# terryye/cuda_FlashAttention

Measured on AMD Instinct MI355X. Metric: FA2 fwd+bwd TFLOP/s at (B=4,H=16,N=8192,d=128); % MFMA peak, higher is better.
Workload: dtype bf16; 1 GPU; FA2 forward+backward bf16, (B=4,H=16,N=8192,d=128) per GPU, non-causal (BASELINE configs[2]); flops = 14 B H N^2 d; B=4, H=16, N=8192, d=128, parallelism=head-sharded replicas x1

## Files before the change

cuda_flashattention_amd/csrc/fa2_bwd_bf16.hip:

```cpp
#include <type_traits>

#include "fa2_regfile.h"
#include "fa2_launch.h"

namespace fa2 {

constexpr float kNoKeyRC = -1.0e30f;
constexpr float kNoKeyLq = 1.0e30f;

template <int D>
__global__ void __launch_bounds__(256) fa2_bwd_delta_kernel(const __bf16* __restrict__ dO,
                                                            const __bf16* __restrict__ O,
                                                            const float* __restrict__ L,
                                                            float* __restrict__ Dv, float* __restrict__ RC,
                                                            size_t rows, int nq, int q_hs, int q_row0, size_t rc_plane,
                                                            float inv_scale)
{
    const size_t r = ((size_t)blockIdx.x * 256 + threadIdx.x) >> 4;
    const int sub = threadIdx.x & 15;
    const size_t head = r / (size_t)nq, i = r % (size_t)nq;
    const size_t row = head * (size_t)q_hs + i;
    const size_t prow = row + (size_t)q_row0;
    float acc = 0.0f;
    if (r < rows) {
#pragma unroll
        for (int c = sub * 8; c < D; c += 128) {
            const bf16x8 a = *reinterpret_cast<const bf16x8*>(dO + row * D + c);
            const bf16x8 b = *reinterpret_cast<const bf16x8*>(O + row * D + c);
#pragma unroll
            for (int e = 0; e < 8; ++e) acc += (float)a[e] * (float)b[e];
        }
    }
#pragma unroll
    for (int off = 8; off >= 1; off >>= 1) acc += __shfl_xor(acc, off, 16);
    if (r < rows && sub == 0) {
        Dv[prow] = acc;
        const float l = L[row];
        RC[prow] = l == -INFINITY ? kNoKeyRC : -l * inv_scale;
        RC[rc_plane + prow] = -acc;
    }
}

constexpr int kBwdRows = 256;
constexpr int kDqWaves = 4;
constexpr int kDqKV = 64;
constexpr int kDkQ = 32;

typedef __attribute__((address_space(3))) void* lptr_t;

#include "fa2_bwd_dq_body.inc"

#define FA2_DQ_CLOBBERS "memory", "vcc", FA2_RF512
#define FA2_DQ_OPS_128 [r0] "v"(roff[0]), [r1] "v"(roff[1]), [r2] "v"(roff[2]), [r3] "v"(roff[3]), [r4] "v"(roff[4]), [r5] "v"(roff[5]), \
    [r6] "v"(roff[6]), [r7] "v"(roff[7]), [t0] "v"(toff[0]), [t1] "v"(toff[1]), [t2] "v"(toff[2]), [t3] "v"(toff[3]), [t4] "v"(toff[4]),     \
    [t5] "v"(toff[5]), [t6] "v"(toff[6]), [t7] "v"(toff[7])
#define FA2_DQ_OPS_64 [r0] "v"(roff[0]), [r1] "v"(roff[1]), [r2] "v"(roff[2]), [r3] "v"(roff[3]), [t0] "v"(toff[0]), [t1] "v"(toff[1]),    \
    [t2] "v"(toff[2]), [t3] "v"(toff[3])

constexpr int kBwdRegFile = RF512;

template <int D, int BUF, bool MASKED>
__device__ __forceinline__ void dq_body(const uint32_t (&roff)[D / 16], const uint32_t (&toff)[D / 16], float c2, float lq0, float lq1,
                                        const f32x16& nd0, const f32x16& nd1, int hi0, int hi1, int hp0, int hp1)
{
#define FA2_DQ_CASE(DD, B, M)                                                                                                      \
    if constexpr (D == DD && BUF == B && MASKED == bool(M))                                                                          \
        asm volatile(FA2_DQ_BODY_D##DD##_B##B##_M##M : : FA2_DQ_OPS_##DD, [c2] "s"(c2), [lq0] "v"(lq0), [lq1] "v"(lq1), [nd0] "v"(nd0), \
                     [nd1] "v"(nd1), [hi0] "v"(hi0), [hi1] "v"(hi1), [hp0] "v"(hp0), [hp1] "v"(hp1) : FA2_DQ_CLOBBERS);
    FA2_DQ_CASE(128, 0, 0) FA2_DQ_CASE(128, 1, 0) FA2_DQ_CASE(128, 2, 0) FA2_DQ_CASE(128, 0, 1) FA2_DQ_CASE(128, 1, 1) FA2_DQ_CASE(128, 2, 1)
    FA2_DQ_CASE(64, 0, 0) FA2_DQ_CASE(64, 1, 0) FA2_DQ_CASE(64, 2, 0) FA2_DQ_CASE(64, 0, 1) FA2_DQ_CASE(64, 1, 1) FA2_DQ_CASE(64, 2, 1)
// ... 361 lines not shown
        } else {
            dkdv_body<D, buf, 0, false>(roff, toff, rcadr, c2, 0, 0, 0);
            dkdv_body<D, buf, 1, false>(roff, toff, rcadr, c2, 0, 0, 0);
        }
    };

    for (int t = t0; t < tend; t += 2) {
        tile(std::integral_constant<int, 0>{}, t);
        tile(std::integral_constant<int, 1>{}, t + 1);
    }
    }

    asm volatile("s_waitcnt lgkmcnt(0)" ::: "memory");
    mfma_acc_settle();
    static_for<2>([&](auto KB) {
        constexpr int kb = decltype(KB)::value;
        const int key = kw0 + 32 * kb + ki;
        char* dKk = (char*)p.dK + slab + (size_t)(key < N ? key : 0) * ROWB;
        char* dVk = (char*)p.dV + slab + (size_t)(key < N ? key : 0) * ROWB;
        static_for<4 * DT>([&](auto G) {
            constexpr int dt = decltype(G)::value / 4, g = decltype(G)::value % 4;
            constexpr int RK = A_DK + 16 * (kb * DT + dt) + 4 * g, RV = A_DV + 16 * (kb * DT + dt) + 4 * g;
            bf16x4 a, b;
            a[0] = (__bf16)(aread<RK>() * p.scale); a[1] = (__bf16)(aread<RK + 1>() * p.scale);
            a[2] = (__bf16)(aread<RK + 2>() * p.scale); a[3] = (__bf16)(aread<RK + 3>() * p.scale);
            b[0] = (__bf16)aread<RV>(); b[1] = (__bf16)aread<RV + 1>();
            b[2] = (__bf16)aread<RV + 2>(); b[3] = (__bf16)aread<RV + 3>();
            if (key < N) {
                *reinterpret_cast<bf16x4*>(dKk + 2 * (32 * dt + 8 * g + 4 * h)) = a;
                *reinterpret_cast<bf16x4*>(dVk + 2 * (32 * dt + 8 * g + 4 * h)) = b;
            }
        });
    });
}

template <int D, bool CAUSAL>
__global__ void __launch_bounds__(256, 1) __attribute__((amdgpu_num_vgpr(60))) fa2_bwd_dkdv_kernel(BwdArgs p)
{
    const int ncb = (p.Nk + kDkKeys - 1) / kDkKeys;
    int kvhead, cb;
    map_block(blockIdx.x, p.BH / p.kv_group, ncb, kvhead, cb);
    bwd_dkdv_impl<D, CAUSAL>(p, kvhead, cb);
}

template <int D, bool CAUSAL>
__global__ void __launch_bounds__(256, 1) __attribute__((amdgpu_num_vgpr(60))) fa2_bwd_dkdv_varlen_kernel(VarlenBwdArgs v)
{
    int kvhead, idx;
    map_block(blockIdx.x, v.a.BH / v.a.kv_group, v.n_key_items, kvhead, idx);
    const VarlenItem it = uniform_item(v.key_items, idx);
    bwd_dkdv_impl<D, CAUSAL>(bwd_varlen_view<D>(v.a, it), kvhead, it.block);
}

template <int D, bool CAUSAL>
static hipError_t launch_bwd_one(const BwdArgs& a, hipStream_t stream)
{
    const size_t rows = (size_t)a.BH * a.Nq;
    hipError_t e = hipSuccess;
    if (a.phases & 1) {
        hipLaunchKernelGGL((fa2_bwd_delta_kernel<D>), dim3((unsigned)((rows * 16 + 255) / 256)), dim3(256), 0,
                           stream, (const __bf16*)a.dO, (const __bf16*)a.O, a.L, a.D, a.RC, rows, a.Nq, a.q_hs, a.q_row0,
                           (size_t)a.BH * a.q_hs, 1.0f / a.scale);
        e = hipGetLastError();
        if (e != hipSuccess) return e;
    }
    const int nb = (a.Nq + kBwdRows - 1) / kBwdRows;
    constexpr int lds_dq = 3 * 2 * kDqKV * D * 2;
    constexpr int lds_dk = kDkKeys * D * 2 + 2 * (2 * 2 * kDkQ * D * 2 + 512);
    if (a.phases & 2) {
        e = launch_lds<fa2_bwd_dq_kernel<D, CAUSAL>>(dim3((unsigned)(nb * a.BH)), dim3(256), lds_dq, stream, a);
        if (e != hipSuccess) return e;
    }
    if (a.phases & 4) {
        const int ncb = (a.Nk + kDkKeys - 1) / kDkKeys;
        e = launch_lds<fa2_bwd_dkdv_kernel<D, CAUSAL>>(dim3((unsigned)(ncb * (a.BH / a.kv_group))), dim3(256), lds_dk, stream, a);
    }
    return e;
}

template <int D, bool CAUSAL>
static hipError_t launch_bwd_varlen_one(const VarlenBwdArgs& v, hipStream_t stream)
{
    const BwdArgs& a = v.a;
    const size_t rows = (size_t)a.BH * a.q_hs;
    hipLaunchKernelGGL((fa2_bwd_delta_kernel<D>), dim3((unsigned)((rows * 16 + 255) / 256)), dim3(256), 0, stream,
                       (const __bf16*)a.dO, (const __bf16*)a.O, a.L, a.D, a.RC, rows, a.q_hs, a.q_hs, 0, rows, 1.0f / a.scale);
    hipError_t e = hipGetLastError();
    if (e != hipSuccess) return e;
    constexpr int lds_dq = 3 * 2 * kDqKV * D * 2;
    constexpr int lds_dk = kDkKeys * D * 2 + 2 * (2 * 2 * kDkQ * D * 2 + 512);
    e = launch_lds<fa2_bwd_dq_varlen_kernel<D, CAUSAL>>(dim3((unsigned)(v.n_row_items * a.BH)), dim3(256), lds_dq, stream, v);
    if (e != hipSuccess) return e;
    return launch_lds<fa2_bwd_dkdv_varlen_kernel<D, CAUSAL>>(dim3((unsigned)(v.n_key_items * (a.BH / a.kv_group))), dim3(256), lds_dk,
                                                            stream, v);
}

hipError_t launch_bwd_varlen_bf16(const VarlenBwdArgs& v, hipStream_t stream)
{
    const BwdArgs& a = v.a;
    if (a.kv_group < 1 || a.BH % a.kv_group != 0 || v.n_row_items < 1 || v.n_key_items < 1 || !v.row_items || !v.key_items)
        return hipErrorInvalidValue;
    if (a.d == 128) return a.causal ? launch_bwd_varlen_one<128, true>(v, stream) : launch_bwd_varlen_one<128, false>(v, stream);
    if (a.d == 64) return a.causal ? launch_bwd_varlen_one<64, true>(v, stream) : launch_bwd_varlen_one<64, false>(v, stream);
    return hipErrorInvalidValue;
}

hipError_t launch_bwd_bf16(const BwdArgs& a, hipStream_t stream)
{
    if (a.kv_group < 1 || a.BH % a.kv_group != 0) return hipErrorInvalidValue;
    if (a.d == 128) return a.causal ? launch_bwd_one<128, true>(a, stream) : launch_bwd_one<128, false>(a, stream);
    if (a.d == 64) return a.causal ? launch_bwd_one<64, true>(a, stream) : launch_bwd_one<64, false>(a, stream);
    return hipErrorInvalidValue;
}

}
```

cuda_flashattention_amd/csrc/fa2_bwd_fused.hip:

```cpp
#include <cstdlib>
#include <cstring>
#include <type_traits>

#include "fa2_regfile.h"
#include "fa2_launch.h"

namespace fa2 {

#include "fa2_bwd_fused_body.inc"

typedef __attribute__((address_space(3))) void* fused_lptr_t;

#ifndef FA2_FUSED_DSKEY
#define FA2_FUSED_DSKEY(row) (((row) >> 1) & 7)
#endif

#ifndef FA2_FUSED_DIAG
#define FA2_FUSED_DIAG 0
#endif

constexpr int kFusedRegFile = RF512;

#define FA2_FUSED_CLOBBERS "memory", "vcc", FA2_RF512
#define FA2_FUSED_OPS_128 [r0] "v"(roff[0]), [r1] "v"(roff[1]), [r2] "v"(roff[2]), [r3] "v"(roff[3]), [r4] "v"(roff[4]), [r5] "v"(roff[5]),  \
    [r6] "v"(roff[6]), [r7] "v"(roff[7]), [t0] "v"(toff[0]), [t1] "v"(toff[1]), [t2] "v"(toff[2]), [t3] "v"(toff[3]), [t4] "v"(toff[4]),   \
    [t5] "v"(toff[5]), [t6] "v"(toff[6]), [t7] "v"(toff[7]), [rc] "v"(rcv), [c2] "s"(c2)
#define FA2_FUSED_OPS_64 [r0] "v"(roff[0]), [r1] "v"(roff[1]), [r2] "v"(roff[2]), [r3] "v"(roff[3]), [t0] "v"(toff[0]), [t1] "v"(toff[1]),    \
    [t2] "v"(toff[2]), [t3] "v"(toff[3]), [rc] "v"(rcv), [c2] "s"(c2)

struct FusedStep {
    __amdgpu_buffer_rsrc_t drs, lrs, qrs, grs, rcrs, ctl;
    uint32_t dso, lso, qso, rcso, pvo, mso;
    int need, pval;
};
#define FA2_FUSED_STEP(TEXT, DD, ...)                                                                                                 \
    asm volatile(TEXT                                                                                                                 \
                 : [err] "+s"(err)                                                                                                    \
                 : FA2_FUSED_OPS_##DD, [vm] "i"(VMW), [dqv] "v"(dqv), [drs] "s"(f.drs), [dso] "s"(f.dso), [lrs] "s"(f.lrs), [lso] "s"(f.lso), \
                   [mw] "s"(mw), [mw2] "s"(mw2), [qrs] "s"(f.qrs), [grs] "s"(f.grs), [rcrs] "s"(f.rcrs), [qso] "s"(f.qso),               \
                   [rcso] "s"(f.rcso), [dvo] "v"(dvo), [rcvo] "v"(rcvo), [wv] "s"(wv), [ctl] "s"(f.ctl), [pvo] "s"(f.pvo),               \
                   [mso] "s"(f.mso), [need] "s"(f.need), [pval] "s"(f.pval) __VA_ARGS__                                                \
                 : FA2_FUSED_CLOBBERS, "s12", "s13", "scc", "exec", "m0", "v39")
template <int D, int BUF, int PAR, int VMW, bool MASKED>
__device__ __forceinline__ void fused_cbody(const uint32_t (&roff)[D / 16], const uint32_t (&toff)[D / 16], uint32_t rcv, float c2, uint32_t dqv,
                                            uint32_t dvo, uint32_t rcvo, uint32_t mw, uint32_t mw2, int wv, const FusedStep& f, int& err,
                                            int lo0 = 0, int lo1 = 0)
{
#define FA2_FUSED_CASE(TAG, DD, B, P)                                                                                                 \
    if constexpr (D == DD && BUF == B && PAR == P && MASKED) FA2_FUSED_STEP(FA2_FUSED##TAG##_MBODY_B##B##_P##P, DD, , [lo0] "v"(lo0), [lo1] "v"(lo1)); \
    if constexpr (D == DD && BUF == B && PAR == P && !MASKED) FA2_FUSED_STEP(FA2_FUSED##TAG##_CBODY_B##B##_P##P, DD);
#define FA2_FUSED_CASES(TAG, DD) \
    FA2_FUSED_CASE(TAG, DD, 0, 0) FA2_FUSED_CASE(TAG, DD, 0, 1) FA2_FUSED_CASE(TAG, DD, 1, 0) FA2_FUSED_CASE(TAG, DD, 1, 1) FA2_FUSED_CASE(TAG, DD, 2, 0) FA2_FUSED_CASE(TAG, DD, 2, 1)
    FA2_FUSED_CASES(, 128) FA2_FUSED_CASES(64, 64)
#undef FA2_FUSED_CASES
#undef FA2_FUSED_CASE
}

template <int BUF, int PAR, int VMW>
__device__ __forceinline__ void fused_body(const uint32_t (&roff)[8], const uint32_t (&toff)[8], uint32_t rcv, float c2)
{
#define FA2_FUSED_CASE(B, P) \
    if constexpr (BUF == B && PAR == P) asm volatile(FA2_FUSED_BODY_B##B##_P##P : : FA2_FUSED_OPS_128, [vm] "i"(VMW) : FA2_FUSED_CLOBBERS);
    FA2_FUSED_CASE(0, 0) FA2_FUSED_CASE(0, 1) FA2_FUSED_CASE(1, 0) FA2_FUSED_CASE(1, 1) FA2_FUSED_CASE(2, 0) FA2_FUSED_CASE(2, 1)
#undef FA2_FUSED_CASE
}

template <int DQT>
__device__ __forceinline__ void fused_dq_atomic(__amdgpu_buffer_rsrc_t rs, uint32_t voff, uint32_t soff)
{
    asm volatile(
        "s_add_u32 s12, %2, 4096\n\ts_add_u32 s13, %2, 8192\n\ts_add_u32 s14, %2, 12288\n\t"
// ... 52 lines not shown
constexpr int g_hook_fault = 0, g_hook_grid = 0;
#define FA2_HOOK_NOTE_GRID(n) ((void)0)
#endif

__device__ __forceinline__ int fused_ctl_ints(int BH, int ncb) { return kCtlHeadmap + 16 * (BH + kHmPad) + 9 * BH * ncb; }

__device__ __forceinline__ int fused_load_sc1(const int* p)
{
    int v;
    asm volatile("global_load_dword %0, %1, off sc1\n\ts_waitcnt vmcnt(0)" : "=v"(v) : "v"(p) : "memory");
    return v;
}
__device__ __forceinline__ void fused_seen_set(int v)
{
    asm volatile("v_mov_b32 v39, %0" : : "s"(v) : "v39");
}

__device__ __forceinline__ int fused_lane_id() { return (int)__builtin_amdgcn_mbcnt_hi(~0u, __builtin_amdgcn_mbcnt_lo(~0u, 0u)); }
template <int OFF>
__device__ __forceinline__ int fused_mail_read(uint32_t lds_addr)
{
    int v;
    asm volatile("v_mov_b32 %0, %1\n\tds_read_b32 %0, %0 offset:%c2\n\ts_waitcnt lgkmcnt(0)" : "=&v"(v) : "s"(lds_addr), "i"(OFF) : "memory");
    return __builtin_amdgcn_readfirstlane(v);
}

__device__ __forceinline__ void fused_store_flag(int* p, int v)
{
    asm volatile("global_store_dword %0, %1, off" : : "v"(p), "v"(v) : "memory");
}

__device__ __forceinline__ bool fused_spin_over(int* ctl, int spins)
{
    if (spins > kSpinLimit) {
        atomicExch(ctl + kCtlError, 1);
        return true;
    }
    return (spins & 1023) == 0 && fused_load_sc1(ctl + kCtlError) != 0;
}

template <bool CHAIN, bool CAUSAL, bool RAGGED = false, bool RECT = false, int HD = 128>
__global__ void __launch_bounds__(256, 1) __attribute__((amdgpu_num_vgpr(39))) fa2_bwd_fused_kernel(FusedArgs fp)
{
    static_assert(CHAIN || !RAGGED, "the atomics form has no ragged variant");
    static_assert(!RECT || (CHAIN && !CAUSAL && !RAGGED), "rectangular blocks: chained, unmasked, aligned");
    static_assert(HD == 128 || (HD == 64 && CHAIN && !RECT), "head_dim 64: chained, square");
    extern __shared__ __attribute__((aligned(16))) char smem[];
    const BwdArgs& p = fp.b;
    constexpr int D = HD, ROWB = 2 * D, KS = D / 16, DT = D / 32;
    constexpr int DQW = 128;
    constexpr int TROWS = 32;
    constexpr bool W = D == 128;
    constexpr int QRING = W ? FA2_FUSED_QRING : FA2_FUSED64_QRING, BUFB = W ? FA2_FUSED_BUFB : FA2_FUSED64_BUFB,
                  DSB = W ? FA2_FUSED_DSB : FA2_FUSED64_DSB, LDSB = W ? FA2_FUSED_LDS : FA2_FUSED64_LDS;
    constexpr int CPR = D / 8, RPI = 64 / CPR, NINS = TROWS / RPI;
    constexpr int VF = W ? FA2_FUSED_VF : FA2_FUSED64_VF, DQT = W ? FA2_FUSED_DQT : FA2_FUSED64_DQT,
                  ROFFK = W ? FA2_FUSED_ROFFK : FA2_FUSED64_ROFFK, DSWR = W ? FA2_FUSED_DSWR : FA2_FUSED64_DSWR,
                  DSRD = W ? FA2_FUSED_DSRD : FA2_FUSED64_DSRD, KT = W ? FA2_FUSED_KT : FA2_FUSED64_KT;
    constexpr int VMW = CHAIN ? (W ? 4 : 2) : 63;
    int* const mail = reinterpret_cast<int*>(smem + LDSB);
    const uint32_t mail_addr = __builtin_amdgcn_readfirstlane((uint32_t)(uintptr_t)smem) + LDSB;

    const int tid = threadIdx.x;
    const int lane = tid & 63;
    const int wave = __builtin_amdgcn_readfirstlane(tid >> 6);
    const int ki = lane & 31;
    const int h = lane >> 5;
    const int N = p.Nk;
    const int NP = RAGGED ? fp.npad : N;
    const int NQ = RECT ? p.Nq : N;
    const int NPQ = RECT ? NQ : NP;
    const int QHS = RECT ? p.q_hs : N, KHS = RECT ? p.k_hs : N;
    const int QR0 = RECT ? p.q_row0 : 0;
    const int ncb = NP / 256;
    const int ntiles = NPQ / TROWS;
    const int niter = ((ntiles + 1 + 5) / 6) * 6;
    const float c2 = p.scale * kLog2e;
    const size_t rc_plane = (size_t)p.BH * (RECT ? QHS : NP);

    const uint32_t lbase = (uint32_t)(uintptr_t)smem;
    const int trq = (lane & 15) >> 2, trp = lane & 3, trcb = (lane >> 4) & 1;
    uint32_t roff[KS], toff[2 * DT];
#pragma unroll
    for (int s = 0; s < KS; ++s) roff[s] = lbase + QRING + lds_off<D>(ki, 2 * s + h);
#pragma unroll
    for (int dt = 0; dt < DT; ++dt)
#pragma unroll
        for (int jj = 0; jj < 2; ++jj)
            toff[2 * dt + jj] = lbase + QRING + lds_off<D>(8 * jj + 4 * h + trq, 4 * dt + 2 * trcb + (trp >> 1)) + 8 * (trp & 1);
    const uint32_t rcv = lbase + QRING + 2 * TROWS * ROWB + 16 * h;
    static_for<KS>([&](auto S) {
        constexpr int sidx = decltype(S)::value;
        vset<kFusedRegFile, CL_TOP, ROFFK + sidx>(lbase + lds_off<D>(ki + 64 * wave, 2 * sidx + h));
    });
    const int ecol = W ? wave : (wave & 1), ekey0 = W ? 0 : 128 * (wave >> 1);
    static_for<2>([&](auto JJ) {
        constexpr int jj = decltype(JJ)::value;
        vset<kFusedRegFile, CL_TOP, KT + jj>(lbase + ekey0 * ROWB + lds_off<D>(8 * jj + 4 * h + trq, 4 * ecol + 2 * trcb + (trp >> 1)) + 8 * (trp & 1));
        const int row = 8 * jj + 4 * h + trq;
        vset<kFusedRegFile, CL_TOP, DSRD + jj>(lbase + DSB + (ekey0 + row) * 64 + 8 * ((4 * trcb + trp) ^ FA2_FUSED_DSKEY(row)));
    });
    static_for<4>([&](auto C) {
        constexpr int c = decltype(C)::value;
        vset<kFusedRegFile, CL_TOP, DSWR + c>(lbase + DSB + (64 * wave + ki) * 64 + 8 * (((2 * c) | h) ^ FA2_FUSED_DSKEY(ki)));
    });
    const int doff = lds_dma_off<D>(wave * RPI, lane);
    const uint32_t dqv = CHAIN ? (uint32_t)(wave * 4096 + lane * 16) : (uint32_t)(((4 * h) * D + 32 * wave + ki) * 4);
// ... 64 lines not shown

    auto next_unit_loads = [&]() {
        if constexpr (CHAIN) {
            take_ticket();
            __syncthreads();
            const int hn = fused_mail_read<0>(mail_addr);
            if (hn >= 0) issue_unit_loads(hn, fused_mail_read<4>(mail_addr));
        }
    };
    next_unit_loads();

    for (;;) {
#ifdef FA2_FUSED_STATS
        const uint64_t s_pull = __builtin_readcyclecounter();
#endif
        int head, cb, err0 = 0;
        if constexpr (CHAIN) {
            head = fused_mail_read<0>(mail_addr);
            cb = fused_mail_read<4>(mail_addr);
            err0 = fused_mail_read<8>(mail_addr);
            if (head < 0) break;
        } else {
            map_block(blockIdx.x, p.BH, ncb, head, cb);
            issue_unit_loads(head, cb);
        }
        const size_t slab = (size_t)head * QHS * ROWB;
        const char* Qh = (const char*)p.Q + slab;
        const char* Gh = (const char*)p.dO + slab;
        const int kw0 = cb * 256 + wave * 64;
        {
            const u32x4 z = {0u, 0u, 0u, 0u};
            static_for<4 * DT>([&](auto T) { azero16<kFusedRegFile, CL_ACC, 16 * decltype(T)::value>(z); });
        }

        const auto q_rsrc = __builtin_amdgcn_make_buffer_rsrc((void*)Qh, 0, NQ * ROWB, 0x00020000);
        const auto g_rsrc = __builtin_amdgcn_make_buffer_rsrc((void*)Gh, 0, NQ * ROWB, 0x00020000);
        const int rcoff = (int)(((wave == 0 ? 0 : rc_plane) + (size_t)head * (RECT ? QHS : NP) + QR0 + (fused_lane_id() & 31)) * 4);
        auto stage = [&](int t, int buf) {
            char* b = smem + QRING + buf * BUFB;
#pragma unroll
            for (int j = wave; j < 2 * NINS; j += 4) {
                const int which = j / NINS, piece = j % NINS;
                const int soff = (t * TROWS + piece * RPI) * ROWB;
                __builtin_amdgcn_raw_ptr_buffer_load_lds(which ? g_rsrc : q_rsrc, (fused_lptr_t)(b + which * (TROWS * ROWB) + piece * 1024),
                                                         16, doff, soff, 0, 0);
            }
            if (wave < 2 && fused_lane_id() < 32)
                __builtin_amdgcn_raw_ptr_buffer_load_lds(rc_rsrc, (fused_lptr_t)(b + 2 * TROWS * ROWB + wave * 128), 4, rcoff, t * TROWS * 4, 0, 0);
        };
        const int n_u = CAUSAL ? ntiles - 8 * cb : ntiles;
        const int niter_u = CAUSAL ? ((n_u + 1 + 5) / 6) * 6 : niter;
        const bool ragged_unit = RAGGED && !CAUSAL && cb == ncb - 1;
        const int first_masked = CAUSAL ? ((n_u - 8) / 6) * 6 : (ragged_unit ? 0 : niter_u);
        auto tl = [&](int u) { return CAUSAL ? ntiles - 1 - u : u; };
        stage(tl(0), 0);
#ifdef FA2_FUSED_PREFILL
        stage(tl(1), 1);
        stage(tl(2), 2);
#endif
        fused_dq_zero<DQT>();
        asm volatile("s_waitcnt vmcnt(0)" ::: "memory");
        __syncthreads();
        if constexpr (W) asm volatile(FA2_FUSED_PRO : : FA2_FUSED_OPS_128, [vm] "i"(VMW) : FA2_FUSED_CLOBBERS);
        else asm volatile(FA2_FUSED64_PRO : : FA2_FUSED_OPS_64, [vm] "i"(VMW) : FA2_FUSED_CLOBBERS);

        const auto dq_rsrc = __builtin_amdgcn_make_buffer_rsrc((void*)(fp.dQacc + (size_t)head * NPQ * DQW), 0, NPQ * DQW * 4, 0x00020000);
        int* const mine = prog_base + head * ncb + cb;
        const int* const prev = mine - 1;
        const int prev_off = (int)((prev - fp.ctl) * 4);
        const int mine_off = (int)((mine - fp.ctl) * 4);
        if constexpr (CHAIN) fused_seen_set(0);
        int err = err0;
#ifdef FA2_FUSED_STATS
        int st_steps = 0, st_polls = 0, st_cycles = 0;
        const uint64_t u0 = __builtin_readcyclecounter();
#endif

        const auto null_rsrc = __builtin_amdgcn_make_buffer_rsrc((void*)fp.dQacc, 0, 0, 0x00020000);
        const bool hp_unit = cb > 0;
        const auto lrs_unit = hp_unit && !(FA2_FUSED_DIAG & 2) ? dq_rsrc : null_rsrc;
        auto step = [&](auto BUF, auto PAR, auto MASKED, auto FAST_, int t) {
            constexpr int buf = decltype(BUF)::value, par = decltype(PAR)::value;
            constexpr bool masked = decltype(MASKED)::value;
            constexpr bool FAST = decltype(FAST_)::value;
            if constexpr (CHAIN && FAST) {
                FusedStep f;
                f.drs = dq_rsrc;
                f.lrs = lrs_unit;
                f.dso = (uint32_t)(tl(t - 1) * TROWS * DQW * 4);
                f.lso = (uint32_t)(tl(t) * TROWS * DQW * 4);
                f.qrs = q_rsrc; f.grs = g_rsrc; f.rcrs = rc_rsrc; f.ctl = ctl_rsrc;
                f.qso = (uint32_t)(tl(t + 1) * TROWS * ROWB + wave * 1024);
                f.rcso = (uint32_t)(tl(t + 1) * TROWS * 4);
                f.pvo = (uint32_t)prev_off; f.mso = (uint32_t)mine_off;
                f.need = (hp_unit && !err && !(FA2_FUSED_DIAG & 1)) ? t + 1 : (int)0x80000000;
                f.pval = t;
#ifdef FA2_TEST_HOOKS
                if (fp.fault && cb == 1) f.pval = 0;
#endif
                fused_cbody<D, buf, par, VMW, false>(roff, toff, rcv, c2, dqv, (uint32_t)doff, (uint32_t)rcoff, lbase + QRING + wave * 1024,
                                                  lbase + QRING + wave * 128, wave, f, err, 0, 0);
            } else if constexpr (CHAIN) {
                FusedStep f;
                const bool live = t >= 1 && t <= n_u;
                const bool more = t + 1 < n_u;
                const bool has_prev = t < n_u && cb > 0;
                f.drs = live ? dq_rsrc : null_rsrc;
                f.lrs = has_prev && !(FA2_FUSED_DIAG & 2) ? dq_rsrc : null_rsrc;
                f.dso = (uint32_t)__builtin_amdgcn_readfirstlane(tl(t - 1) * TROWS * DQW * 4);
                f.lso = (uint32_t)__builtin_amdgcn_readfirstlane(tl(t) * TROWS * DQW * 4);
                f.qrs = q_rsrc; f.grs = g_rsrc; f.rcrs = rc_rsrc; f.ctl = ctl_rsrc;
                f.qso = more ? (uint32_t)(tl(t + 1) * TROWS * ROWB + wave * 1024) : 0x40000000u;
                f.rcso = more ? (uint32_t)(tl(t + 1) * TROWS * 4) : 0x40000000u;
                f.pvo = (uint32_t)prev_off; f.mso = (uint32_t)mine_off;
                f.need = (has_prev && !err && !(FA2_FUSED_DIAG & 1)) ? t + 1 : (int)0x80000000;
                f.pval = t < n_u ? t : n_u;
#ifdef FA2_TEST_HOOKS
                if (fp.fault && cb == 1) f.pval = 0;
#endif
                int lo0 = 0, lo1 = 0;
                if constexpr (masked) {
                    const int lane_m = (int)__builtin_amdgcn_mbcnt_hi(~0u, __builtin_amdgcn_mbcnt_lo(~0u, 0u));
                    if constexpr (CAUSAL) {
                        lo0 = kw0 + (lane_m & 31) - 4 * (lane_m >> 5) - TROWS * tl(t);
                        lo1 = lo0 + 32;
                    } else {
                        lo0 = kw0 + (lane_m & 31) < N ? -0x40000000 : 0x40000000;
                        lo1 = kw0 + 32 + (lane_m & 31) < N ? -0x40000000 : 0x40000000;
                    }
                }
#ifdef FA2_FUSED_STATS2
                const uint64_t b0 = __builtin_readcyclecounter();
#endif
                fused_cbody<D, buf, par, VMW, masked>(roff, toff, rcv, c2, dqv, (uint32_t)doff, (uint32_t)rcoff, lbase + QRING + wave * 1024,
                                                   lbase + QRING + wave * 128, wave, f, err, lo0, lo1);
#ifdef FA2_FUSED_STATS2
                st_cycles += (int)(__builtin_readcyclecounter() - b0);
#endif
            } else {
                static_assert(W || CHAIN, "head_dim 64: chained form only");
                stage(t + 1, (buf + 1) % 3);
                if constexpr (W) fused_body<buf, par, VMW>(roff, toff, rcv, c2);
#ifndef FA2_FUSED_NO_DQ
                if (t >= 1 && t <= ntiles) fused_dq_atomic<DQT>(dq_rsrc, dqv, (uint32_t)__builtin_amdgcn_readfirstlane((t - 1) * TROWS * D * 4));
#endif
                fused_dq_zero<DQT>();
            }
        };
        auto six = [&](auto MASKED, auto FAST_, int t) {
            step(std::integral_constant<int, 0>{}, std::integral_constant<int, 0>{}, MASKED, FAST_, t);
            step(std::integral_constant<int, 1>{}, std::integral_constant<int, 1>{}, MASKED, FAST_, t + 1);
            step(std::integral_constant<int, 2>{}, std::integral_constant<int, 0>{}, MASKED, FAST_, t + 2);
            step(std::integral_constant<int, 0>{}, std::integral_constant<int, 1>{}, MASKED, FAST_, t + 3);
            step(std::integral_constant<int, 1>{}, std::integral_constant<int, 0>{}, MASKED, FAST_, t + 4);
            step(std::integral_constant<int, 2>{}, std::integral_constant<int, 1>{}, MASKED, FAST_, t + 5);
        };
        const int fast_end = CHAIN ? n_u - 2 : -1;
        {
            const int plain_end = first_masked;
            int t = 0;
            asm volatile("" : "+s"(t));
            if (t < plain_end) { six(std::false_type{}, std::false_type{}, t); t += 6; }
#pragma unroll 1
            for (; t + 5 <= fast_end && t < plain_end; t += 6) six(std::false_type{}, std::true_type{}, t);
#pragma unroll 1
            for (; t < plain_end; t += 6) six(std::false_type{}, std::false_type{}, t);
            if constexpr (CHAIN && (CAUSAL || RAGGED)) {
#pragma unroll 1
                for (; t < niter_u; t += 6) six(std::true_type{}, std::false_type{}, t);
            }
        }
        asm volatile("s_waitcnt vmcnt(0) lgkmcnt(0)" ::: "memory");
        if constexpr (CHAIN)
            if (err && !err0 && wave == 0 && fused_lane_id() == 0) atomicExch(fp.ctl + kCtlError, 1);
#ifdef FA2_FUSED_STATS
        const uint64_t s_loop = __builtin_readcyclecounter();
#endif
        next_unit_loads();

        mfma_acc_settle();
        const int lane_ep = (int)__builtin_amdgcn_mbcnt_hi(~0u, __builtin_amdgcn_mbcnt_lo(~0u, 0u));
        const int ki_ep = lane_ep & 31, h_ep = lane_ep >> 5;
        static_for<2>([&](auto KB) {
            constexpr int kb = decltype(KB)::value;
            const int key = kw0 + 32 * kb + ki_ep;
            const size_t slab_k = RECT ? (size_t)head * KHS * ROWB : slab;
            char* const dKb = (char*)p.dK + slab_k;
            char* const dVb = (char*)p.dV + slab_k;
            const uint32_t koff = (uint32_t)key * ROWB + 16u * h_ep;
            char* dKk = dKb + koff;
            char* dVk = dVb + koff;
            static_for<2 * DT>([&](auto G) {
                constexpr int dt = decltype(G)::value / 2, gp = decltype(G)::value % 2;
                constexpr int RK = 16 * (kb * DT + dt) + 8 * gp, RV = 32 * DT + RK;
                auto pack4 = [&](float a, float b, float c, float d, float sc) {
                    bf16x4 v;
                    v[0] = (__bf16)(a * sc); v[1] = (__bf16)(b * sc); v[2] = (__bf16)(c * sc); v[3] = (__bf16)(d * sc);
                    return __builtin_bit_cast(u32x2, v);
                };
                auto emit = [&](u32x2 x, u32x2 y, char* dst) {
                    const auto s0 = __builtin_amdgcn_permlane32_swap(x[0], y[0], false, false);
                    const auto s1 = __builtin_amdgcn_permlane32_swap(x[1], y[1], false, false);
                    const u32x4 o = {s0[0], s1[0], s0[1], s1[1]};
#ifdef FA2_FUSED_ST_NT
                    if (!RAGGED || key < N) __builtin_nontemporal_store(o, reinterpret_cast<u32x4*>(dst + 2 * (32 * dt + 16 * gp)));
#else
                    if (!RAGGED || key < N) *reinterpret_cast<u32x4*>(dst + 2 * (32 * dt + 16 * gp)) = o;
#endif
                };
                emit(pack4(aread<RK>(), aread<RK + 1>(), aread<RK + 2>(), aread<RK + 3>(), p.scale),
                     pack4(aread<RK + 4>(), aread<RK + 5>(), aread<RK + 6>(), aread<RK + 7>(), p.scale), dKk);
                emit(pack4(aread<RV>(), aread<RV + 1>(), aread<RV + 2>(), aread<RV + 3>(), 1.0f),
                     pack4(aread<RV + 4>(), aread<RV + 5>(), aread<RV + 6>(), aread<RV + 7>(), 1.0f), dVk);
            });
        });
#ifdef FA2_FUSED_STATS
        if (CHAIN && wave == 0 && fused_lane_id() == 0) {
            atomicAdd(fp.ctl + kCtlError + 1, st_steps);
            atomicAdd(fp.ctl + kCtlError + 2, st_polls);
            atomicAdd((unsigned long long*)(fp.ctl + kCtlError + 4), (unsigned long long)st_cycles);
            atomicAdd((unsigned long long*)(fp.ctl + kCtlError + 6), (unsigned long long)(__builtin_readcyclecounter() - u0));
            int* rec = prog_base + p.BH * ncb + 8 * (head * ncb + cb);
            rec[0] = xcc; rec[1] = st_cycles; rec[2] = (int)(u0 - s_pull); rec[3] = (int)(__builtin_readcyclecounter() - s_loop);
            *(unsigned long long*)(rec + 4) = u0; *(unsigned long long*)(rec + 6) = __builtin_readcyclecounter();
        }
#endif
        if constexpr (!CHAIN) break;
    }
}

__global__ void __launch_bounds__(256) fa2_bwd_fused_dq_out_kernel(const float* __restrict__ acc, __bf16* __restrict__ dQ, size_t n8, float scale,
                                                                    const int* __restrict__ err)
{
    const float poison = (err && *err) ? __builtin_nanf("") : 0.0f;
    const size_t stride = (size_t)gridDim.x * 256;
    for (size_t i = (size_t)blockIdx.x * 256 + threadIdx.x; i < n8; i += stride) {
        const f32x4 a = reinterpret_cast<const f32x4*>(acc)[2 * i], b = reinterpret_cast<const f32x4*>(acc)[2 * i + 1];
        bf16x8 o;
#pragma unroll
        for (int e = 0; e < 4; ++e) { o[e] = (__bf16)(a[e] * scale + poison); o[4 + e] = (__bf16)(b[e] * scale + poison); }
        reinterpret_cast<bf16x8*>(dQ)[i] = o;
    }
}

__global__ void __launch_bounds__(256) fa2_bwd_fused_dq_out_chain_kernel(const float* __restrict__ acc, __bf16* __restrict__ dQ, size_t n4, float scale,
                                                                          const int* __restrict__ err, int N, int NP, int qhs)
{
    const float poison = *err ? __builtin_nanf("") : 0.0f;
    const size_t stride = (size_t)gridDim.x * 256;
    const size_t tiles = (size_t)(NP / 32);
    for (size_t i = (size_t)blockIdx.x * 256 + threadIdx.x; i < n4; i += stride) {
        const f32x4 a = reinterpret_cast<const f32x4*>(acc)[i];
        const int lane = (int)(i & 63), g = (int)((i >> 6) & 3), wave = (int)((i >> 8) & 3);
        const size_t tg = i >> 10, head = tg / tiles;
        const int row = (int)(tg % tiles) * 32 + 8 * g + 4 * (lane >> 5);
        __bf16* o = dQ + (head * (size_t)qhs + row) * 128 + 32 * wave + (lane & 31);
#pragma unroll
        for (int e = 0; e < 4; ++e)
            if (row + e < N) o[(size_t)e * 128] = (__bf16)(a[e] * scale + poison);
    }
}

__global__ void __launch_bounds__(256) fa2_bwd_fused_dq_out_chain64_kernel(const float* __restrict__ acc, __bf16* __restrict__ dQ, size_t n4h, float scale,
                                                                            const int* __restrict__ err, int N, int NP)
{
    const float poison = *err ? __builtin_nanf("") : 0.0f;
    const size_t stride = (size_t)gridDim.x * 256;
    const size_t tiles = (size_t)(NP / 32);
// ... 46 lines not shown
    int dev = 0;
    if (hipGetDevice(&dev) != hipSuccess || dev < 0 || dev >= 64) { if (why) *why = "no current device"; return false; }
    if (!verdict[dev]) {
        hipDeviceProp_t pr;
        if (hipGetDeviceProperties(&pr, dev) != hipSuccess) { if (why) *why = "device properties unavailable"; return false; }
        verdict[dev] = strncmp(pr.gcnArchName, "gfx950", 6) != 0 ? 2 : pr.multiProcessorCount != 256 ? 3 : 1;
    }
    static const char* const text[] = {"", "single five-product kernel (gfx950, 256 CUs: the layout the ordered hand-off was validated on)",
                                       "two kernels: device is not gfx950", "two kernels: device does not expose 256 CUs (partitioned GPU): "
                                       "the ordered hand-off was validated in SPX mode only"};
    if (why) *why = text[verdict[dev]];
    return verdict[dev] == 1;
}

hipError_t bwd_fused_read_error(const int* ctl, int* err, hipStream_t stream)
{
    hipError_t e = hipMemcpyAsync(err, ctl + kCtlError, sizeof(int), hipMemcpyDeviceToHost, stream);
    if (e != hipSuccess) return e;
    return hipStreamSynchronize(stream);
}

hipError_t bwd_fused_clear_error(int* ctl, hipStream_t stream)
{
    return launch_fill_f32(reinterpret_cast<float*>(ctl + kCtlError), 1, 0.0f, stream);
}

size_t bwd_fused_kvpart_bytes(int BH, int N, int d) { return (size_t)2 * BH * N * d * 2; }
size_t bwd_fused_ctl_bytes(int BH, int N) { return (size_t)(kCtlHeadmap + 16 * (BH + kHmPad) + 9 * BH * ((N + 255) / 256)) * sizeof(int); }

template <int HD>
static hipError_t launch_chained_square(bool causal, bool ragged, dim3 grid, int lds, hipStream_t stream, const FusedArgs& fa)
{
    if (causal)
        return ragged ? launch_lds<fa2_bwd_fused_kernel<true, true, true, false, HD>>(grid, dim3(256), lds, stream, fa)
                      : launch_lds<fa2_bwd_fused_kernel<true, true, false, false, HD>>(grid, dim3(256), lds, stream, fa);
    return ragged ? launch_lds<fa2_bwd_fused_kernel<true, false, true, false, HD>>(grid, dim3(256), lds, stream, fa)
                  : launch_lds<fa2_bwd_fused_kernel<true, false, false, false, HD>>(grid, dim3(256), lds, stream, fa);
}

hipError_t launch_bwd_fused_bf16(const BwdArgs& a, float* dQacc, int* ctl, int mode, hipStream_t stream, float* rcpad, void* kvpart)
{
    const int npad = (a.Nk + 255) / 256 * 256;
    const bool ragged = npad != a.Nk;
    const bool rect = a.Nq != a.Nk || a.q_hs != a.Nq || a.k_hs != a.Nk || a.q_row0 != 0;
    if ((a.d != 128 && a.d != 64) || a.Nk < 1 || a.Nq < 1) return hipErrorInvalidValue;
    if (a.d == 64 && (mode != 1 || rect)) return hipErrorInvalidValue;
    if (rect && (mode != 1 || a.causal || ragged || a.Nq % 32 != 0 || a.q_row0 < 0 || a.q_hs < a.q_row0 + a.Nq || a.k_hs < a.Nk))
        return hipErrorInvalidValue;
    if (ragged && (mode != 1 || !rcpad)) return hipErrorInvalidValue;
    const bool grouped = a.kv_group > 1;
    if (a.kv_group < 1 || a.BH % a.kv_group != 0 || (grouped && (mode != 1 || rect || !kvpart))) return hipErrorInvalidValue;
    if (a.causal && (mode != 1 || a.causal_shift != 0)) return hipErrorInvalidValue;
    hipError_t e = hipSuccess;
    if (a.phases & 1) {
        BwdArgs d = a;
        d.phases = 1;
        e = launch_bwd_bf16(d, stream);
        if (e != hipSuccess) return e;
    }
    if (!(a.phases & 8)) return hipSuccess;
    const size_t elems = (size_t)a.BH * (rect ? a.Nq : npad) * 128;
    const int units = a.BH * (npad / 256);
    if (ragged) {
        const size_t n = (size_t)2 * a.BH * npad;
        hipLaunchKernelGGL(fa2_bwd_fused_rcpad_kernel, dim3((unsigned)((n + 255) / 256)), dim3(256), 0, stream, (const float*)a.RC, rcpad,
                           a.BH, a.Nk, npad);
        e = hipGetLastError();
        if (e != hipSuccess) return e;
    }
    FusedArgs fa{a, dQacc, ctl, npad, ragged ? (const float*)rcpad : (const float*)a.RC, g_hook_fault};
    const size_t part_elems = (size_t)a.BH * a.Nk * a.d;
    if (grouped) {
        fa.b.dK = kvpart;
        fa.b.dV = (__bf16*)kvpart + part_elems;
    }
    const int lds = (a.d == 64 ? FA2_FUSED64_LDS : FA2_FUSED_LDS) + 16;
    if (mode == 0) {
        e = launch_fill_f32(dQacc, elems, 0.0f, stream);
        if (e != hipSuccess) return e;
        e = bwd_fused_clear_error(ctl, stream);
        if (e != hipSuccess) return e;
        e = launch_lds<fa2_bwd_fused_kernel<false, false>>(dim3((unsigned)units), dim3(256), lds, stream, fa);
    } else {
        static int cus[64] = {};
        int dev = 0;
        e = hipGetDevice(&dev);
        if (e != hipSuccess) return e;
        if (dev < 0 || dev >= 64) return hipErrorInvalidDevice;
        if (!cus[dev]) {
            e = hipDeviceGetAttribute(&cus[dev], hipDeviceAttributeMultiprocessorCount, dev);
            if (e != hipSuccess) return e;
        }
        e = launch_fill_f32(reinterpret_cast<float*>(ctl), bwd_fused_ctl_bytes(a.BH, a.Nk) / sizeof(float), 0.0f, stream);
        if (e != hipSuccess) return e;
        int avail = cus[dev] - (a.reserve_cus > 0 ? a.reserve_cus : 0);
        if (avail < 1) avail = 1;
        int wgs = units < avail ? units : avail;
        if (g_hook_grid >= 1 && g_hook_grid < wgs) wgs = g_hook_grid;
        FA2_HOOK_NOTE_GRID(wgs);
        const dim3 grid((unsigned)wgs);
        if (rect)
            e = launch_lds<fa2_bwd_fused_kernel<true, false, false, true>>(grid, dim3(256), lds, stream, fa);
        else
            e = a.d == 64 ? launch_chained_square<64>(a.causal, ragged, grid, lds, stream, fa)
                          : launch_chained_square<128>(a.causal, ragged, grid, lds, stream, fa);
    }
    if (e != hipSuccess) return e;
    if (mode == 0)
        hipLaunchKernelGGL(fa2_bwd_fused_dq_out_kernel, dim3(2048), dim3(256), 0, stream, dQacc, (__bf16*)a.dQ, elems / 8, a.scale,
                           (const int*)nullptr);
    else if (a.d == 64)
        hipLaunchKernelGGL(fa2_bwd_fused_dq_out_chain64_kernel, dim3(4096), dim3(256), 0, stream, dQacc, (__bf16*)a.dQ, elems / 8, a.scale,
                           ctl + kCtlError, a.Nk, npad);
    else
        hipLaunchKernelGGL(fa2_bwd_fused_dq_out_chain_kernel, dim3(4096), dim3(256), 0, stream, dQacc, (__bf16*)a.dQ, elems / 4, a.scale,
                           ctl + kCtlError, rect ? a.Nq : a.Nk, rect ? a.Nq : npad, rect ? a.q_hs : a.Nk);
    e = hipGetLastError();
    if (e != hipSuccess || !grouped) return e;
    hipLaunchKernelGGL(fa2_bwd_fused_dkdv_out_kernel, dim3(4096), dim3(256), 0, stream, (const bf16x8*)fa.b.dK, (const bf16x8*)fa.b.dV,
                       (bf16x8*)a.dK, (bf16x8*)a.dV, (size_t)a.Nk * a.d / 8, (size_t)(a.BH / a.kv_group), a.kv_group);
    return hipGetLastError();
}

}
```

cuda_flashattention_amd/csrc/fa2_launch.h:

```cpp
#pragma once
#include <hip/hip_runtime.h>
#include <stddef.h>

namespace fa2 {

struct FwdArgs {
    const void* Q;
    const void* K;
    const void* V;
    void* O;
    float* L;
    float* Oacc;
    float* M;
    int BH, Nq, Nk, d;
    float scale;
    int causal;
    int causal_shift;
    int resume;
    int finalize;
    int q_hs, k_hs;
    int kv_group;
};

hipError_t launch_fwd1_bf16(const FwdArgs& a, hipStream_t stream);

struct VarlenItem {
    int q_row0, k_row0;
    int len_q, len_k;
    int block;
};
struct VarlenFwdArgs { FwdArgs a; const VarlenItem* items; int n_items; };
hipError_t launch_fwd1_varlen_bf16(const VarlenFwdArgs& v, hipStream_t stream);
hipError_t launch_accumulate_bf16(float* acc, const void* src, size_t rows, size_t cols, size_t pitch, int init, hipStream_t stream);
hipError_t launch_finalize_state(const float* Oacc, const float* M, float* L, void* O, size_t rows, int d, hipStream_t stream);

struct FwdFp8Args {
    const void* Q; const void* K; const void* V;
    void* Vt;
    float* kn;
    void* O;
    float* L;
    int BH, N, Npad, d;
    float scale;
    int causal;
    float o_scale;
};
hipError_t launch_fwd_fp8(const FwdFp8Args& a, hipStream_t stream);

struct BwdArgs {
    const void* Q; const void* K; const void* V; const void* O; const void* dO;
    const float* L;
    void* dQ; void* dK; void* dV;
    float* D;
    float* RC;
    int BH, Nq, Nk, d;
    int q_hs, k_hs;
    int q_row0;
    float scale;
    int causal;
    int causal_shift;
    int phases;
    int reserve_cus;
    int kv_group;
};

hipError_t launch_bwd_bf16(const BwdArgs& a, hipStream_t stream);
struct VarlenBwdArgs {
    BwdArgs a;
    const VarlenItem* row_items; const VarlenItem* key_items;
    int n_row_items, n_key_items;
};
hipError_t launch_bwd_varlen_bf16(const VarlenBwdArgs& v, hipStream_t stream);
size_t bwd_fused_ctl_bytes(int BH, int N);
size_t bwd_fused_kvpart_bytes(int BH, int N, int d);
hipError_t launch_bwd_fused_bf16(const BwdArgs& a, float* dQacc, int* ctl, int mode, hipStream_t stream, float* rcpad = nullptr,
                                 void* kvpart = nullptr);
bool bwd_fused_device_ok(const char** why);
hipError_t bwd_fused_read_error(const int* ctl, int* err, hipStream_t stream);
hipError_t bwd_fused_clear_error(int* ctl, hipStream_t stream);

struct F32Args {
    const float* Q; const float* K; const float* V; float* O; float* L;
    const float* dO; float* dQ; float* dK; float* dV; float* D;
    int BH, N, d;
    float scale;
    int causal;
    int phases;
    int Nk;
    float* M;
    int resume, finalize;
};
hipError_t launch_fwd_f32(const F32Args& a, hipStream_t stream);
hipError_t launch_bwd_f32(const F32Args& a, hipStream_t stream);

template <auto K, typename A>
inline hipError_t launch_lds(dim3 grid, dim3 block, int lds, hipStream_t stream, const A& arg)
{
    static bool done[64] = {};
    int dev = 0;
    hipError_t e = hipGetDevice(&dev);
    if (e != hipSuccess) return e;
    if (dev < 0 || dev >= 64) return hipErrorInvalidDevice;
    if (!done[dev]) {
        e = hipFuncSetAttribute(reinterpret_cast<const void*>(K), hipFuncAttributeMaxDynamicSharedMemorySize, lds);
        if (e != hipSuccess) return e;
        done[dev] = true;
    }
    hipLaunchKernelGGL(K, grid, block, lds, stream, arg);
    return hipGetLastError();
}

hipError_t launch_fa1_f32(const float* Q, const float* K, const float* V, float* O, float* l, float* m, int N, int d, int Bc,
                          hipStream_t stream);

hipError_t launch_fill_f32(float* p, size_t n, float value, hipStream_t stream);
hipError_t launch_mfma_probe(const void* in, float* out, int iters, int blocks, hipStream_t stream);
hipError_t launch_f32_to_bf16(const float* src, void* dst, size_t n, hipStream_t stream);
hipError_t launch_bf16_to_f32(const void* src, float* dst, size_t n, hipStream_t stream);
hipError_t launch_read_clocks(unsigned long long* out, hipStream_t stream);
// ... 3 lines not shown
```

Before: 1311 TFLOP/s.

## Stage fused bwd dK/dV epilogue through LDS and trim tail steps

Rewrites the fused backward kernel's dK/dV epilogue so each wave first packs its accumulators to bf16 with a vector convert, writes them to a swizzled LDS staging area, then reads them back so that global stores become row-contiguous 16-byte writes. The tail six-step group of the chain loop now skips steps beyond the live tile count instead of running padding steps. An optional path (off by default) lets the delta kernel zero the control buffer with extra blocks, removing the separate fill launch. The LDS staging adds a barrier in the non-chain path and extra LDS traffic, and reuses the dS tile region, which must be free at that point.

```diff
diff --git a/cuda_flashattention_amd/csrc/fa2_bwd_bf16.hip b/cuda_flashattention_amd/csrc/fa2_bwd_bf16.hip
--- a/cuda_flashattention_amd/csrc/fa2_bwd_bf16.hip
+++ b/cuda_flashattention_amd/csrc/fa2_bwd_bf16.hip
@@ -7,6 +7,7 @@
 
 constexpr float kNoKeyRC = -1.0e30f;
 constexpr float kNoKeyLq = 1.0e30f;
+constexpr unsigned kDeltaZeroBlocks = 32;
 
 template <int D>
 __global__ void __launch_bounds__(256) fa2_bwd_delta_kernel(const __bf16* __restrict__ dO,
@@ -14,8 +15,14 @@
                                                             const float* __restrict__ L,
                                                             float* __restrict__ Dv, float* __restrict__ RC,
                                                             size_t rows, int nq, int q_hs, int q_row0, size_t rc_plane,
-                                                            float inv_scale)
-{
+                                                            float inv_scale, unsigned row_blocks, float* __restrict__ zero,
+                                                            size_t nzero)
+{
+    if (blockIdx.x >= row_blocks) {
+        for (size_t i = (size_t)(blockIdx.x - row_blocks) * 256 + threadIdx.x; i < nzero; i += (size_t)(gridDim.x - row_blocks) * 256)
+            zero[i] = 0.0f;
+        return;
+    }
     const size_t r = ((size_t)blockIdx.x * 256 + threadIdx.x) >> 4;
     const int sub = threadIdx.x & 15;
     const size_t head = r / (size_t)nq, i = r % (size_t)nq;
@@ -483,16 +490,24 @@
     bwd_dkdv_impl<D, CAUSAL>(bwd_varlen_view<D>(v.a, it), kvhead, it.block);
 }
 
+template <int D>
+static hipError_t launch_delta(const BwdArgs& a, float* zero, size_t nzero, hipStream_t stream)
+{
+    const size_t rows = (size_t)a.BH * a.Nq;
+    const unsigned row_blocks = (unsigned)((rows * 16 + 255) / 256);
+    hipLaunchKernelGGL((fa2_bwd_delta_kernel<D>), dim3(row_blocks + (nzero ? kDeltaZeroBlocks : 0u)), dim3(256), 0, stream,
+                       (const __bf16*)a.dO, (const __bf16*)a.O, a.L, a.D, a.RC, rows, a.Nq, a.q_hs, a.q_row0, (size_t)a.BH * a.q_hs,
+                       1.0f / a.scale, row_blocks, zero, nzero);
+    return hipGetLastError();
+}
+
 template <int D, bool CAUSAL>
 static hipError_t launch_bwd_one(const BwdArgs& a, hipStream_t stream)
 {
     const size_t rows = (size_t)a.BH * a.Nq;
     hipError_t e = hipSuccess;
     if (a.phases & 1) {
-        hipLaunchKernelGGL((fa2_bwd_delta_kernel<D>), dim3((unsigned)((rows * 16 + 255) / 256)), dim3(256), 0,
-                           stream, (const __bf16*)a.dO, (const __bf16*)a.O, a.L, a.D, a.RC, rows, a.Nq, a.q_hs, a.q_row0,
-                           (size_t)a.BH * a.q_hs, 1.0f / a.scale);
-        e = hipGetLastError();
+        e = launch_delta<D>(a, nullptr, 0, stream);
         if (e != hipSuccess) return e;
     }
     const int nb = (a.Nq + kBwdRows - 1) / kBwdRows;
@@ -514,8 +529,9 @@
 {
     const BwdArgs& a = v.a;
     const size_t rows = (size_t)a.BH * a.q_hs;
-    hipLaunchKernelGGL((fa2_bwd_delta_kernel<D>), dim3((unsigned)((rows * 16 + 255) / 256)), dim3(256), 0, stream,
-                       (const __bf16*)a.dO, (const __bf16*)a.O, a.L, a.D, a.RC, rows, a.q_hs, a.q_hs, 0, rows, 1.0f / a.scale);
+    const unsigned row_blocks = (unsigned)((rows * 16 + 255) / 256);
+    hipLaunchKernelGGL((fa2_bwd_delta_kernel<D>), dim3(row_blocks), dim3(256), 0, stream, (const __bf16*)a.dO, (const __bf16*)a.O, a.L,
+                       a.D, a.RC, rows, a.q_hs, a.q_hs, 0, rows, 1.0f / a.scale, row_blocks, (float*)nullptr, (size_t)0);
     hipError_t e = hipGetLastError();
     if (e != hipSuccess) return e;
     constexpr int lds_dq = 3 * 2 * kDqKV * D * 2;
@@ -536,6 +552,13 @@
     return hipErrorInvalidValue;
 }
 
+hipError_t launch_bwd_delta_bf16(const BwdArgs& a, float* zero, size_t nzero, hipStream_t stream)
+{
+    if (a.d == 128) return launch_delta<128>(a, zero, nzero, stream);
+    if (a.d == 64) return launch_delta<64>(a, zero, nzero, stream);
+    return hipErrorInvalidValue;
+}
+
 hipError_t launch_bwd_bf16(const BwdArgs& a, hipStream_t stream)
 {
     if (a.kv_group < 1 || a.BH % a.kv_group != 0) return hipErrorInvalidValue;
diff --git a/cuda_flashattention_amd/csrc/fa2_bwd_fused.hip b/cuda_flashattention_amd/csrc/fa2_bwd_fused.hip
--- a/cuda_flashattention_amd/csrc/fa2_bwd_fused.hip
+++ b/cuda_flashattention_amd/csrc/fa2_bwd_fused.hip
@@ -17,6 +17,18 @@
 
 #ifndef FA2_FUSED_DIAG
 #define FA2_FUSED_DIAG 0
+#endif
+#ifndef FA2_FUSED_EPI_LDS
+#define FA2_FUSED_EPI_LDS 1
+#endif
+#ifndef FA2_FUSED_EPI_CVT_PK
+#define FA2_FUSED_EPI_CVT_PK 1
+#endif
+#ifndef FA2_FUSED_EXACT_STEPS
+#define FA2_FUSED_EXACT_STEPS 1
+#endif
+#ifndef FA2_FUSED_DELTA_ZERO
+#define FA2_FUSED_DELTA_ZERO 0
 #endif
 
 constexpr int kFusedRegFile = RF512;
@@ -175,7 +187,8 @@
     constexpr int TROWS = 32;
     constexpr bool W = D == 128;
     constexpr int QRING = W ? FA2_FUSED_QRING : FA2_FUSED64_QRING, BUFB = W ? FA2_FUSED_BUFB : FA2_FUSED64_BUFB,
-                  DSB = W ? FA2_FUSED_DSB : FA2_FUSED64_DSB, LDSB = W ? FA2_FUSED_LDS : FA2_FUSED64_LDS;
+                  DSB = W ? FA2_FUSED_DSB : FA2_FUSED64_DSB, LDSB = W ? FA2_FUSED_LDS : FA2_FUSED64_LDS,
+                  DSTILE = W ? FA2_FUSED_DSTILE : FA2_FUSED64_DSTILE;
     constexpr int CPR = D / 8, RPI = 64 / CPR, NINS = TROWS / RPI;
     constexpr int VF = W ? FA2_FUSED_VF : FA2_FUSED64_VF, DQT = W ? FA2_FUSED_DQT : FA2_FUSED64_DQT,
                   ROFFK = W ? FA2_FUSED_ROFFK : FA2_FUSED64_ROFFK, DSWR = W ? FA2_FUSED_DSWR : FA2_FUSED64_DSWR,
@@ -346,6 +359,7 @@
         const int niter_u = CAUSAL ? ((n_u + 1 + 5) / 6) * 6 : niter;
         const bool ragged_unit = RAGGED && !CAUSAL && cb == ncb - 1;
         const int first_masked = CAUSAL ? ((n_u - 8) / 6) * 6 : (ragged_unit ? 0 : niter_u);
+        const int nlive = n_u + 1;
         auto tl = [&](int u) { return CAUSAL ? ntiles - 1 - u : u; };
         stage(tl(0), 0);
 #ifdef FA2_FUSED_PREFILL
@@ -441,27 +455,29 @@
                 fused_dq_zero<DQT>();
             }
         };
-        auto six = [&](auto MASKED, auto FAST_, int t) {
+        auto six = [&](auto MASKED, auto FAST_, auto LAST_, int t) {
+            constexpr bool LAST = decltype(LAST_)::value;
             step(std::integral_constant<int, 0>{}, std::integral_constant<int, 0>{}, MASKED, FAST_, t);
-            step(std::integral_constant<int, 1>{}, std::integral_constant<int, 1>{}, MASKED, FAST_, t + 1);
-            step(std::integral_constant<int, 2>{}, std::integral_constant<int, 0>{}, MASKED, FAST_, t + 2);
-            step(std::integral_constant<int, 0>{}, std::integral_constant<int, 1>{}, MASKED, FAST_, t + 3);
-            step(std::integral_constant<int, 1>{}, std::integral_constant<int, 0>{}, MASKED, FAST_, t + 4);
-            step(std::integral_constant<int, 2>{}, std::integral_constant<int, 1>{}, MASKED, FAST_, t + 5);
+            if (!LAST || t + 1 < nlive) step(std::integral_constant<int, 1>{}, std::integral_constant<int, 1>{}, MASKED, FAST_, t + 1);
+            if (!LAST || t + 2 < nlive) step(std::integral_constant<int, 2>{}, std::integral_constant<int, 0>{}, MASKED, FAST_, t + 2);
+            if (!LAST || t + 3 < nlive) step(std::integral_constant<int, 0>{}, std::integral_constant<int, 1>{}, MASKED, FAST_, t + 3);
+            if (!LAST || t + 4 < nlive) step(std::integral_constant<int, 1>{}, std::integral_constant<int, 0>{}, MASKED, FAST_, t + 4);
+            if (!LAST || t + 5 < nlive) step(std::integral_constant<int, 2>{}, std::integral_constant<int, 1>{}, MASKED, FAST_, t + 5);
         };
         const int fast_end = CHAIN ? n_u - 2 : -1;
         {
             const int plain_end = first_masked;
+            constexpr std::bool_constant<CHAIN && FA2_FUSED_EXACT_STEPS != 0> last{};
             int t = 0;
             asm volatile("" : "+s"(t));
-            if (t < plain_end) { six(std::false_type{}, std::false_type{}, t); t += 6; }
+            if (t < plain_end) { six(std::false_type{}, std::false_type{}, std::false_type{}, t); t += 6; }
 #pragma unroll 1
-            for (; t + 5 <= fast_end && t < plain_end; t += 6) six(std::false_type{}, std::true_type{}, t);
+            for (; t + 5 <= fast_end && t < plain_end; t += 6) six(std::false_type{}, std::true_type{}, std::false_type{}, t);
 #pragma unroll 1
-            for (; t < plain_end; t += 6) six(std::false_type{}, std::false_type{}, t);
+            for (; t < plain_end; t += 6) six(std::false_type{}, std::false_type{}, last, t);
             if constexpr (CHAIN && (CAUSAL || RAGGED)) {
 #pragma unroll 1
-                for (; t < niter_u; t += 6) six(std::true_type{}, std::false_type{}, t);
+                for (; t < niter_u; t += 6) six(std::true_type{}, std::false_type{}, last, t);
             }
         }
         asm volatile("s_waitcnt vmcnt(0) lgkmcnt(0)" ::: "memory");
@@ -473,12 +489,74 @@
         next_unit_loads();
 
         mfma_acc_settle();
+        const size_t slab_k = RECT ? (size_t)head * KHS * ROWB : slab;
+        auto pack4 = [&](float a, float b, float c, float d, float sc) {
+#if FA2_FUSED_EPI_CVT_PK
+            const f32x4 t = {a * sc, b * sc, c * sc, d * sc};
+            return __builtin_bit_cast(u32x2, __builtin_convertvector(t, bf16x4));
+#else
+            bf16x4 v;
+            v[0] = (__bf16)(a * sc); v[1] = (__bf16)(b * sc); v[2] = (__bf16)(c * sc); v[3] = (__bf16)(d * sc);
+            return __builtin_bit_cast(u32x2, v);
+#endif
+        };
+        auto pair_up = [&](u32x2 x, u32x2 y) {
+            const auto s0 = __builtin_amdgcn_permlane32_swap(x[0], y[0], false, false);
+            const auto s1 = __builtin_amdgcn_permlane32_swap(x[1], y[1], false, false);
+            return u32x4{s0[0], s1[0], s0[1], s1[1]};
+        };
+        auto store16 = [&](char* dst, const u32x4& o) {
+            if ((FA2_FUSED_DIAG & 8) && fp.npad >= 0) return;
+#ifdef FA2_FUSED_ST_NT
+            __builtin_nontemporal_store(o, reinterpret_cast<u32x4*>(dst));
+#else
+            *reinterpret_cast<u32x4*>(dst) = o;
+#endif
+        };
+#if FA2_FUSED_EPI_LDS
+        static_assert(DSB % 256 == 0 && DSTILE == 256 * 64 && LDSB == DSB + 2 * DSTILE, "the staging area is the wave's rows of the two dS tiles");
+        if constexpr (!CHAIN) __syncthreads();
+        auto lane_now = [&]() {
+            int l = (int)__builtin_amdgcn_mbcnt_hi(~0u, __builtin_amdgcn_mbcnt_lo(~0u, 0u));
+            asm volatile("" : "+v"(l));
+            return l;
+        };
+        const uint32_t stg = DSB + 4096 * wave;
+        static_for<4>([&](auto RD) {
+            constexpr int kb = decltype(RD)::value / 2, tv = decltype(RD)::value % 2;
+            constexpr int R0 = 32 * DT * tv + 16 * DT * kb;
+            const float sc = tv ? 1.0f : p.scale;
+            {
+                const int lw = lane_now(), ki_w = lw & 31, h_w = lw >> 5;
+                const uint32_t wo = stg + (W ? (ki_w >> 4) * DSTILE + (ki_w & 15) * ROWB : ki_w * ROWB) + 16 * (h_w ^ (ki_w & 7));
+                static_for<2 * DT>([&](auto G) {
+                    constexpr int g = decltype(G)::value, R = R0 + 8 * g;
+                    const u32x4 o = pair_up(pack4(aread<R>(), aread<R + 1>(), aread<R + 2>(), aread<R + 3>(), sc),
+                                            pack4(aread<R + 4>(), aread<R + 5>(), aread<R + 6>(), aread<R + 7>(), sc));
+                    *reinterpret_cast<u32x4*>(smem + (wo ^ (32u * g))) = o;
+                });
+            }
+            asm volatile("s_waitcnt lgkmcnt(0)" ::: "memory");
+            const int lr = lane_now(), rl = lr / CPR, cl = lr % CPR;
+            const uint32_t ro = stg + rl * ROWB + 16 * (cl ^ rl);
+            char* const gb = (char*)(tv ? p.dV : p.dK) + slab_k + (size_t)(kw0 + 32 * kb) * ROWB;
+            const uint32_t goff = 16u * lr;
+            static_for<TROWS / RPI>([&](auto I) {
+                constexpr int r0 = RPI * decltype(I)::value;
+                constexpr uint32_t rb = W ? (r0 >> 4) * DSTILE + (r0 & 15) * ROWB : r0 * ROWB;
+                const u32x4 o = *reinterpret_cast<const u32x4*>(smem + ((ro ^ (16u * (r0 & 7))) + rb));
+                char* const gr = gb + r0 * ROWB;
+                if (!RAGGED || kw0 + 32 * kb + r0 + rl < N) store16(gr + goff, o);
+                if constexpr (decltype(I)::value % 2 == 1) asm volatile("" ::: "memory");
+            });
+            asm volatile("" ::: "memory");
+        });
+#else
         const int lane_ep = (int)__builtin_amdgcn_mbcnt_hi(~0u, __builtin_amdgcn_mbcnt_lo(~0u, 0u));
         const int ki_ep = lane_ep & 31, h_ep = lane_ep >> 5;
         static_for<2>([&](auto KB) {
             constexpr int kb = decltype(KB)::value;
             const int key = kw0 + 32 * kb + ki_ep;
-            const size_t slab_k = RECT ? (size_t)head * KHS * ROWB : slab;
             char* const dKb = (char*)p.dK + slab_k;
             char* const dVb = (char*)p.dV + slab_k;
             const uint32_t koff = (uint32_t)key * ROWB + 16u * h_ep;
@@ -487,20 +565,9 @@
             static_for<2 * DT>([&](auto G) {
                 constexpr int dt = decltype(G)::value / 2, gp = decltype(G)::value % 2;
                 constexpr int RK = 16 * (kb * DT + dt) + 8 * gp, RV = 32 * DT + RK;
-                auto pack4 = [&](float a, float b, float c, float d, float sc) {
-                    bf16x4 v;
-                    v[0] = (__bf16)(a * sc); v[1] = (__bf16)(b * sc); v[2] = (__bf16)(c * sc); v[3] = (__bf16)(d * sc);
-                    return __builtin_bit_cast(u32x2, v);
-                };
                 auto emit = [&](u32x2 x, u32x2 y, char* dst) {
-                    const auto s0 = __builtin_amdgcn_permlane32_swap(x[0], y[0], false, false);
-                    const auto s1 = __builtin_amdgcn_permlane32_swap(x[1], y[1], false, false);
-                    const u32x4 o = {s0[0], s1[0], s0[1], s1[1]};
-#ifdef FA2_FUSED_ST_NT
-                    if (!RAGGED || key < N) __builtin_nontemporal_store(o, reinterpret_cast<u32x4*>(dst + 2 * (32 * dt + 16 * gp)));
-#else
-                    if (!RAGGED || key < N) *reinterpret_cast<u32x4*>(dst + 2 * (32 * dt + 16 * gp)) = o;
-#endif
+                    const u32x4 o = pair_up(x, y);
+                    if (!RAGGED || key < N) store16(dst + 2 * (32 * dt + 16 * gp), o);
                 };
                 emit(pack4(aread<RK>(), aread<RK + 1>(), aread<RK + 2>(), aread<RK + 3>(), p.scale),
                      pack4(aread<RK + 4>(), aread<RK + 5>(), aread<RK + 6>(), aread<RK + 7>(), p.scale), dKk);
@@ -508,6 +575,7 @@
                      pack4(aread<RV + 4>(), aread<RV + 5>(), aread<RV + 6>(), aread<RV + 7>(), 1.0f), dVk);
             });
         });
+#endif
 #ifdef FA2_FUSED_STATS
         if (CHAIN && wave == 0 && fused_lane_id() == 0) {
             atomicAdd(fp.ctl + kCtlError + 1, st_steps);
@@ -660,10 +728,12 @@
     if (a.kv_group < 1 || a.BH % a.kv_group != 0 || (grouped && (mode != 1 || rect || !kvpart))) return hipErrorInvalidValue;
     if (a.causal && (mode != 1 || a.causal_shift != 0)) return hipErrorInvalidValue;
     hipError_t e = hipSuccess;
+    const bool delta_zeroes = FA2_FUSED_DELTA_ZERO && mode == 1 && (a.phases & 1) && (a.phases & 8);
     if (a.phases & 1) {
         BwdArgs d = a;
         d.phases = 1;
-        e = launch_bwd_bf16(d, stream);
+        e = delta_zeroes ? launch_bwd_delta_bf16(d, reinterpret_cast<float*>(ctl), bwd_fused_ctl_bytes(a.BH, a.Nk) / sizeof(float), stream)
+                         : launch_bwd_bf16(d, stream);
         if (e != hipSuccess) return e;
     }
     if (!(a.phases & 8)) return hipSuccess;
@@ -699,7 +769,7 @@
             e = hipDeviceGetAttribute(&cus[dev], hipDeviceAttributeMultiprocessorCount, dev);
             if (e != hipSuccess) return e;
         }
-        e = launch_fill_f32(reinterpret_cast<float*>(ctl), bwd_fused_ctl_bytes(a.BH, a.Nk) / sizeof(float), 0.0f, stream);
+        if (!delta_zeroes) e = launch_fill_f32(reinterpret_cast<float*>(ctl), bwd_fused_ctl_bytes(a.BH, a.Nk) / sizeof(float), 0.0f, stream);
         if (e != hipSuccess) return e;
         int avail = cus[dev] - (a.reserve_cus > 0 ? a.reserve_cus : 0);
         if (avail < 1) avail = 1;
diff --git a/cuda_flashattention_amd/csrc/fa2_launch.h b/cuda_flashattention_amd/csrc/fa2_launch.h
--- a/cuda_flashattention_amd/csrc/fa2_launch.h
+++ b/cuda_flashattention_amd/csrc/fa2_launch.h
@@ -65,6 +65,7 @@
 };
 
 hipError_t launch_bwd_bf16(const BwdArgs& a, hipStream_t stream);
+hipError_t launch_bwd_delta_bf16(const BwdArgs& a, float* zero, size_t nzero, hipStream_t stream);
 struct VarlenBwdArgs {
     BwdArgs a;
     const VarlenItem* row_items; const VarlenItem* key_items;
```

Result: no change. 1308 TFLOP/s (-0.2%).
